# erwincoumans/tiny-differentiable-simulator

Hardware: NVIDIA H100
Metric: env-steps/sec (N parallel sims) (higher is better)
Workload: dtype f32 (ABA, factorisation, PGS) + f64 (kinematics, inertias, CRBA, Jacobians, LCP rhs)

## Files before the change

### tiny-differentiable-simulator_b200/csrc/tds_steps.cu

```cuda
#include <cuda_runtime.h>
#include <stdlib.h>

#include "tds_wcommon.cuh"
#include "tds_team.h"
#include "generated/spec_laikago.h"
#include "generated/spec_ant.h"

namespace tdss {
using namespace tds;
using namespace tdsw;

#ifndef TDS_DENSE_MAX_CAND
#define TDS_DENSE_MAX_CAND 8
#endif
constexpr int TT = TDS_TEAM_T;
constexpr int ST = 32;

template <int V> struct IC { static constexpr int value = V; };
#define CI(...) (IC<(__VA_ARGS__)>::value)
#define CD(...) ([]() { constexpr double cd_v_ = (__VA_ARGS__); return cd_v_; }())
#define CDOT3(ax, ay, az, v)                                                                                            \
  ([&]() {                                                                                                              \
    using T_ = decltype((v).x);                                                                                         \
    constexpr double a_ = (ax), b_ = (ay), c_ = (az);                                                                   \
// ... 171 lines not shown
template <class SP> struct CandTab {
  static constexpr int NC = SP::N_CAND > 0 ? SP::N_CAND : 1;
  int owner[NC], own[NC];
};
template <class SP> constexpr CandTab<SP> make_cand() {
  CandTab<SP> t{};
  for (int g = 0; g < SP::N_CAND; ++g) {
    t.owner[g] = SP::CAND_OWNER[g];
    t.own[g] = (SP::CAND_OWNER[g] == 0 && SP::CAND_LPT[g] < Cls<SP>::n_pts_trunk()) ? 0 : 1;
  }
  return t;
}
template <class SP> __device__ const CandTab<SP>& cand_tab();

template <class SP, typename RA, typename RC, typename RS> struct Lay {
  static constexpr int RAW = sizeof(RA) / 4, RCW = sizeof(RC) / 4, RSW = sizeof(RS) / 4;
  static constexpr int NTD = SP::N_TD, NTRI = NTD * (NTD + 1) / 2, NOD = SP::N_OD_MAX;
  static constexpr int O = 0;
  static constexpr int RB = O + 4 * RCW;
  static constexpr int XWW = ev(12 * RCW + 12 * RAW);
  static constexpr int XW = RB + 10 * RCW;
  static constexpr int TS = XW + (SP::N_XW_TEAM + 1) * XWW;
  static constexpr int TLW = ev(14 * RAW);
  static constexpr int TL = TS + SP::N_TRUNK * 6 * RCW;
  static constexpr int TLR = ev(TL + SP::N_TRUNK * TLW);
  static constexpr int TKS = ev(TLR + trunk_rbi_slot<SP>(SP::N_TRUNK) * 10 * RCW);
  static constexpr int TQD = ev(TKS + 3 * SP::N_TRUNK);
  static constexpr int ACC_IC = ev(27 * RAW);
  static constexpr int ACCW = ev(ACC_IC + 10 * RCW);
  static constexpr int ACC = ev(TQD + NTD);
  static constexpr int PW = ev(NTRI * RSW);
  static constexpr int CONW = ev((3 * (NOD + NTD) + 9) * RSW);
  static constexpr int ACC_SZ = cmax(cmax(TT * cmax(SP::N_ATT, 1) * ACCW, TT * PW), cmax(SP::N_CAND, 1) * CONW);
  static constexpr int LT = ACC + ACC_SZ;
  static constexpr int CON = ACC;
  static constexpr int ZT = ev(LT + NTRI * RSW);
  static constexpr int WO = ev(ZT + NTD * RSW);
  static constexpr int ASTG = ev(WO + TT * NOD * RSW);
  static constexpr int XS = ev(ASTG + SP::N_ACT);
  static constexpr int FLG = ev(XS + (SP::N_CAND > TDS_DENSE_MAX_CAND ? 3 * SP::N_CAND * RSW : 0));
  static constexpr int SHARED = ev(FLG + 2 * TT + 2);
  static constexpr int PRIV = ev(cmax(SP::KMAX - SP::N_TRUNK, 1) * 10 * RCW);
  static constexpr int TOTAL = SHARED + TT * PRIV;
};

template <typename T> TDS_D T* sp(char* base, int lane, int word) {
  return (sizeof(T) == 4) ? ((T*)base) + (size_t)word * ST + lane : ((T*)base) + (size_t)(word >> 1) * ST + lane;
}
template <typename T> TDS_D T negz() { return T(-0.0); }
template <typename T> TDS_D Abi<T> abi_nz() {
  Abi<T> a; const T z = negz<T>();
  a.I = {z, z, z, z, z, z}; a.M = a.I;
// ... 19 lines not shown
  using L = Lay<SP, RA, RC, RS>;
  using C = Cls<SP>;
  static_assert(C::uniform(), "the subtrees of the model are not one structural class (use the table-driven kernel)");
  constexpr bool XOUT = VAR == 0, HOSTIO = VAR == 2;
  constexpr int RAW = L::RAW, RCW = L::RCW;
  constexpr int NT = SP::N_TRUNK, NTD = SP::N_TD, NLOC = SP::N_LOC[0];
  constexpr int NOD = SP::N_OD[0], NODA = cmax(NOD, 1), NTDA = cmax(NTD, 1), NTRI = L::NTRI, NTRIA = cmax(NTRI, 1);
  constexpr int NPO = C::n_pts_own(), NPOA = cmax(NPO, 1), NPTR = C::n_pts_trunk(), NPTRA = cmax(NPTR, 1);
  constexpr int NACCA = cmax(SP::N_ACC, 1), NXLA = cmax(SP::N_XW_LANE, 1), NATT = cmax(SP::N_ATT, 1);
  constexpr bool FLOAT = SP::FLOATING != 0;
  const int lane = tid & 31;
  const int env = tile * 32 + lane;
  const bool live = env < io.n;
  const int e = live ? env : io.n - 1;
  const int ns = io.n_stride;
  const LegTab<SP>& LG = leg_tab<SP>(role);
  char* const priv = smem + (size_t)(L::SHARED + role * L::PRIV) * ST * 4;
  int phase_id = 0;
#define TDSS_PHASE() do { if (io.phase_clk && lane == 0 && tile * 32 < io.n_stride) io.phase_clk[((size_t)tile * TT + role) * 16 + phase_id] = clock64(); ++phase_id; } while (0)
#define TDSS_STAMP(slot) do { if (io.phase_clk && lane == 0 && tile * 32 < io.n_stride) io.phase_clk[((size_t)tile * TT + role) * 16 + (slot)] = clock64(); } while (0)
  TDSS_PHASE();
  auto xw_rc = [&](int slot) { return sp<RC>(smem, lane, L::XW + slot * L::XWW); };
  auto xw_ra = [&](int slot) { return sp<RA>(smem, lane, L::XW + slot * L::XWW + 12 * RCW); };
  auto tl_rbi_slot = [&](int slot) { return sp<RC>(smem, lane, L::TLR + slot * 10 * RCW); };
  auto tl_u = [&](int k) { return sp<RA>(smem, lane, L::TL + k * L::TLW); };
  auto tl_v = [&](int k) { return sp<RA>(smem, lane, L::TL + k * L::TLW + 8 * RAW); };
  auto ts_S = [&](int k) { return sp<RC>(smem, lane, L::TS + k * 6 * RCW); };
  float* const tqd = sp<float>(smem, lane, L::TQD);
  unsigned* const flg = sp<unsigned>(smem, lane, L::FLG);

  float qv[SP::KMAX], qdv[SP::KMAX], tauv[SP::KMAX];
  float bq[7], bqd[6];
  sfor<NT, NLOC>([&](auto Kc) {
    constexpr int k = decltype(Kc)::value;
    if constexpr (!(C::flags(k) & TDS_LF_FIXED)) {
      qv[k] = io.q_in[(size_t)LG.qidx[k - NT] * ns + e];
      qdv[k] = io.qd_in[(size_t)LG.qdidx[k - NT] * ns + e];
      tauv[k] = 0.f;
    }
  });
  if (role == 0) {
    sfor<0, NT>([&](auto Kc) {
      constexpr int k = decltype(Kc)::value;
      if constexpr (!(SP::L_FLAGS[0][k] & TDS_LF_FIXED)) {
        qv[k] = io.q_in[(size_t)CI(SP::L_QIDX[0][k]) * ns + e];
        qdv[k] = io.qd_in[(size_t)CI(SP::L_QDIDX[0][k]) * ns + e];
        tauv[k] = 0.f;
      }
    });
    if constexpr (FLOAT) {
// ... 189 lines not shown
      };
      if constexpr ((fl & TDS_LF_PRISMATIC) != 0) {
        const V3<RC> d = rot_axis();
        pi = axpy(d, qi, pi);
        S.bot = d;
      } else {
        const V3<RC> w = rot_axis();
        if constexpr (jt == TDSJ_REVOLUTE_AXIS) {
          const RC dl = sqrt_t(dot(axv, axv));
          RC s = snv[k] / dl;
          const RC c = csv[k];
          Ri = mul(Ri, quat_to_matrix<RC>(axv.x * s, axv.y * s, axv.z * s, c));
        } else {
          const RC s = snv[k], c = csv[k];
          const V3<RC> cx = col_x(Ri), cy = col_y(Ri), cz = col_z(Ri);
          if constexpr (jt == TDSJ_REVOLUTE_X) set_cols(Ri, cx, axpy(cz, s, cy * c), axpy(cy, -s, cz * c));
          else if constexpr (jt == TDSJ_REVOLUTE_Y) set_cols(Ri, axpy(cz, -s, cx * c), cy, axpy(cx, s, cz * c));
          else set_cols(Ri, axpy(cy, s, cx * c), axpy(cx, -s, cy * c), cz);
        }
        S.top = w;
        S.bot = cross(pi, w);
      }
    }
    if constexpr (TR) st6<RC>(ts_S(k), ST, S); else Sreg[k] = S;
    {
      constexpr bool massless = TR ? (SP::L_RBIC[0][k][0] == 0.0 && SP::L_RBIC[0][k][4] == 0.0 && SP::L_RBIC[0][k][5] == 0.0 && SP::L_RBIC[0][k][6] == 0.0 &&
                                      SP::L_RBIC[0][k][7] == 0.0 && SP::L_RBIC[0][k][8] == 0.0 && SP::L_RBIC[0][k][9] == 0.0)
                                   : C::massless(k);
      if constexpr (!massless) {
        double b[10];
        if constexpr (TR) {
          b[0] = CD(SP::L_RBIC[0][k][0]); b[1] = CD(SP::L_RBIC[0][k][1]); b[2] = CD(SP::L_RBIC[0][k][2]); b[3] = CD(SP::L_RBIC[0][k][3]); b[4] = CD(SP::L_RBIC[0][k][4]);
          b[5] = CD(SP::L_RBIC[0][k][5]); b[6] = CD(SP::L_RBIC[0][k][6]); b[7] = CD(SP::L_RBIC[0][k][7]); b[8] = CD(SP::L_RBIC[0][k][8]); b[9] = CD(SP::L_RBIC[0][k][9]);
        } else {
#pragma unroll
          for (int j = 0; j < 10; ++j) b[j] = LG.rbic[ko][j];
        }
        Rbi<RC> r;
        r.m = RC(b[0]);
        const V3<RC> c = pi + mul(Ri, v3<RC>(RC(b[1]), RC(b[2]), RC(b[3])));
        r.h = c * r.m;
        S3<RA> Icf;
        Icf.xx = RA(b[4]); Icf.xy = RA(b[5]); Icf.xz = RA(b[6]); Icf.yy = RA(b[7]); Icf.yz = RA(b[8]); Icf.zz = RA(b[9]);
        const S3<RA> Irot = rot_sym(cvt<RA>(Ri), Icf);
        r.I.xx = RC(Irot.xx); r.I.xy = RC(Irot.xy); r.I.xz = RC(Irot.xz); r.I.yy = RC(Irot.yy); r.I.yz = RC(Irot.yz); r.I.zz = RC(Irot.zz);
        const RC cc = dot(c, c);
        r.I.xx += r.m * (cc - c.x * c.x); r.I.yy += r.m * (cc - c.y * c.y); r.I.zz += r.m * (cc - c.z * c.z);
        r.I.xy -= r.m * c.x * c.y; r.I.xz -= r.m * c.x * c.z; r.I.yz -= r.m * c.y * c.z;
        if constexpr (TR) st_rbi<RC>(tl_rbi_slot(trunk_rbi_slot<SP>(k)), ST, r);
        else st_rbi<RC>(sp<RC>(priv, lane, ko * 10 * RCW), ST, r);
      }
    }
    Sv<RA> v = vp;
    if constexpr (!(fl & TDS_LF_FIXED)) {
      const RA qdi = RA(qdv[k]);
      const Sv<RA> Sf = cvt_sv<RA>(S);
      v.top = axpy(Sf.top, qdi, v.top);
      v.bot = axpy(Sf.bot, qdi, v.bot);
    }
    if constexpr (TR) st6<RA>(tl_v(k), ST, v); else vreg[k] = v;
    constexpr int xs = SP::L_XW[0][k];
    if constexpr (xs >= 0) {
      if constexpr (TR) { st9<RC>(xw_rc(xs + 1), ST, Ri); st3<RC>(xw_rc(xs + 1) + 9 * ST, ST, pi); st6<RA>(xw_ra(xs + 1), ST, v); }
      else { xwR[xs] = Ri; xwp[xs] = pi; }
    }
    if (want_contacts) {
      if constexpr (TR) emit_trunk_geoms(IC<SP::L_GB[0][k]>{}, IC<SP::L_GE[0][k]>{}, IC<SP::L_CAND[0][k]>{}, IC<SP::L_LPT[0][k]>{}, Ri, pi);
      else emit_own_geoms(IC<k>{}, Ri, pi);
    }
    if constexpr (XOUT) if (io.link_xf && live) {
      int link;
      if constexpr (TR) link = CI(SP::L_LINK[0][k]); else link = LG.link[ko];
      float* o = io.link_xf + (size_t)link * 12 * ns + e;
      o[0] = (float)Ri.xx; o[(size_t)1 * ns] = (float)Ri.xy; o[(size_t)2 * ns] = (float)Ri.xz;
      o[(size_t)3 * ns] = (float)Ri.yx; o[(size_t)4 * ns] = (float)Ri.yy; o[(size_t)5 * ns] = (float)Ri.yz;
      o[(size_t)6 * ns] = (float)Ri.zx; o[(size_t)7 * ns] = (float)Ri.zy; o[(size_t)8 * ns] = (float)Ri.zz;
      o[(size_t)9 * ns] = (float)(pi.x + O.x); o[(size_t)10 * ns] = (float)(pi.y + O.y); o[(size_t)11 * ns] = (float)(pi.z + O.z);
    }
    R_prev = Ri; p_prev = pi; v_prev = v;
// ... 28 lines not shown
          }
        }
      });
    }
    plane_off = DOT_PN(O) - RC(CD(SP::PLANE_C[0]));
    st3<RC>(sO, ST, O); sO[3 * ST] = plane_off;
    if constexpr (FLOAT) st9<RC>(sRb, ST, Rb0);
    R_prev = Rb0;
    p_prev = FLOAT ? v3<RC>(RC(0), RC(0), RC(0)) : v3<RC>(-O.x, -O.y, -O.z);
    if constexpr (FLOAT) {
      const M3<RA> RbA = cvt<RA>(Rb0);
      v_prev.top = mul(RbA, v3<RA>(RA(bqd[0]), RA(bqd[1]), RA(bqd[2])));
      v_prev.bot = mul(RbA, v3<RA>(RA(bqd[3]), RA(bqd[4]), RA(bqd[5])));
    } else { v_prev.top = v3<RA>(RA(0), RA(0), RA(0)); v_prev.bot = v_prev.top; }
    st9<RC>(xw_rc(0), ST, R_prev); st3<RC>(xw_rc(0) + 9 * ST, ST, p_prev); st6<RA>(xw_ra(0), ST, v_prev);
    if (want_contacts) emit_trunk_geoms(IC<SP::GEOM_BEGIN[0]>{}, IC<SP::GEOM_BEGIN[1]>{}, IC<0>{}, IC<0>{}, R_prev, p_prev);
    sfor<0, NT>(pass1);
    TDSS_STAMP(13);
  }
  __syncthreads();
  O = ld3<RC>(sO, ST); plane_off = sO[3 * ST];
  M3<RC> Rb = m3_identity<RC>();
  if constexpr (FLOAT) Rb = ld9<RC>(sRb, ST);
  sfor<NT, NLOC>(pass1);
  flg[(2 * role) * ST] = (unsigned)my_active;
  flg[(2 * role + 1) * ST] = (unsigned)(my_active >> 32);
  if constexpr (HOSTIO) {
#pragma unroll
    for (int j = 0; j < AREG; ++j) {
      const int idx = tid + 32 * TT * j;
      if (idx < NACT_TILE) astg[idx] = areg[j];
    }
  }
  const bool cta_contact = __syncthreads_or(my_active != 0ull) != 0;
  if constexpr (HOSTIO) {
    pd_torques();
    if constexpr (TRUNK_LOOP && !DIRECT_TRUNK) {
      if (role == 0) {
        sfor<0, NT>([&](auto Kc) {
          constexpr int k = decltype(Kc)::value;
          if constexpr (!(SP::L_FLAGS[0][k] & TDS_LF_FIXED)) tk_tau[k * ST] = tauv[k];
        });
      }
    }
  }
  const bool solve = (mode == MODE_FULL) && cta_contact;
// ... 2 lines not shown
  for (int r = 0; r < TT; ++r) team_active |= ((unsigned long long)flg[(2 * r + 1) * ST] << 32) | flg[(2 * r) * ST];
  TDSS_PHASE();

  constexpr int NMKK = NODA * (NODA + 1) / 2, NCM = NODA * NTDA;
  RS Mkk[NMKK];
#ifdef TDS_STEPS_KERNEL_ONLY
  RS Cm_store[NCM];
  RS* const Cm = Cm_store;
#else
  RS Cm[NCM];
#endif
  RS Bm[NTRIA];
#pragma unroll
  for (int i = 0; i < NMKK; ++i) Mkk[i] = RS(0);
#pragma unroll
  for (int i = 0; i < NCM; ++i) Cm[i] = RS(0);
#pragma unroll
  for (int i = 0; i < NTRIA; ++i) Bm[i] = RS(0);
  Sv<RA> Ureg[SP::KMAX]; RA invDreg[SP::KMAX], ureg[SP::KMAX];
  Abi<RA> cA = abi_nz<RA>(); Sv<RA> cP = sv_nz<RA>(); Rbi<RC> cC = rbi_nz<RC>();
  Abi<RA> accA[NACCA]; Sv<RA> accP[NACCA]; Rbi<RC> accC[NACCA];
#pragma unroll
  for (int s = 0; s < NACCA; ++s) { accA[s] = abi_nz<RA>(); accP[s] = sv_nz<RA>(); accC[s] = rbi_nz<RC>(); }
  auto S_of = [&](auto Jc) -> Sv<RC> {
    constexpr int j = decltype(Jc)::value;
    if constexpr (j < NT) return ld6<RC>(ts_S(j), ST); else return Sreg[j];
  };
  auto acc_ptr_ra = [&](int r, int s) { return sp<RA>(smem, lane, L::ACC + (r * NATT + s) * L::ACCW); };
  auto acc_ptr_rc = [&](int r, int s) { return sp<RC>(smem, lane, L::ACC + (r * NATT + s) * L::ACCW + L::ACC_IC); };
  auto pass2 = [&](auto Kc) {
    constexpr int k = decltype(Kc)::value;
    constexpr bool TR = k < NT;
    constexpr int ko = TR ? 0 : k - NT;
    constexpr int fl = TR ? SP::L_FLAGS[0][k] : C::flags(k);
    constexpr bool massless = TR ? (SP::L_RBIC[0][k][0] == 0.0 && SP::L_RBIC[0][k][4] == 0.0 && SP::L_RBIC[0][k][5] == 0.0 && SP::L_RBIC[0][k][6] == 0.0 &&
                                    SP::L_RBIC[0][k][7] == 0.0 && SP::L_RBIC[0][k][8] == 0.0 && SP::L_RBIC[0][k][9] == 0.0)
                                 : C::massless(k);
    Sv<RA> v;
    if constexpr (TR) v = ld6<RA>(tl_v(k), ST); else v = vreg[k];
    Rbi<RC> Ic = rbi_nz<RC>();
    Abi<RA> Ia = abi_nz<RA>();
    Sv<RA> pA = sv_nz<RA>();
    if constexpr (!massless) {
      if constexpr (TR) Ic = ld_rbi<RC>(tl_rbi_slot(trunk_rbi_slot<SP>(k)), ST); else Ic = ld_rbi<RC>(sp<RC>(priv, lane, ko * 10 * RCW), ST);
      const Rbi<RA> rb = cvt_rbi<RA>(Ic);
      Ia = abi_from_rbi(rb);
      pA = cross_mf(v, rbi_mul(rb, v));
    }
    if constexpr ((fl & TDS_TF_CHILD_ADJ) != 0) { abi_add(Ia, cA); pA = pA + cP; rbi_add(Ic, cC); }
    constexpr int as = SP::L_ACC[0][k];
    if constexpr (as >= 0) {
      abi_add(Ia, accA[as]); pA = pA + accP[as]; rbi_add(Ic, accC[as]);
      if constexpr (as < SP::N_ATT) {
        static_assert(TR || k < 0, "attachment accumulators are consumed by trunk links");
        sfor<1, TT>([&](auto Rc_) {
          constexpr int r = decltype(Rc_)::value;
          Abi<RA> sa; Sv<RA> sv_;
          acc_ld27<RA>(acc_ptr_ra(r, as), ST, sa, sv_);
          abi_add(Ia, sa); pA = pA + sv_;
          rbi_add(Ic, ld_rbi<RC>(acc_ptr_rc(r, as), ST));
        });
      }
    }
    Sv<RA> pa = pA;
    if constexpr (!(fl & TDS_LF_FIXED)) {
      const Sv<RC> Sd = S_of(IC<k>{});
      const Sv<RA> S = cvt_sv<RA>(Sd);
      const RA qdj = RA(qdv[k]);
      Sv<RA> vJ; vJ.top = S.top * qdj; vJ.bot = S.bot * qdj;
      const Sv<RA> c = cross_mm(v, vJ);
      const Sv<RA> U = abi_mul(Ia, S);
      const RA D = dot(S, U);
      const RA invD = inv_t(D);
      RA tau = RA(tauv[k]);
      if constexpr (TR) {
        if constexpr (SP::L_SD[0][k][0] != 0.0) tau -= RA(CD(SP::L_SD[0][k][0])) * RA(qv[k]);
        if constexpr (SP::L_SD[0][k][1] != 0.0) tau -= RA(CD(SP::L_SD[0][k][1])) * qdj;
      } else {
        if constexpr (C::has_sd(k, 0)) tau -= RA(LG.sd[ko][0]) * RA(qv[k]);
        if constexpr (C::has_sd(k, 1)) tau -= RA(LG.sd[ko][1]) * qdj;
      }
      const RA u = tau - dot(S, pA);
      if constexpr (TR) { st6<RA>(tl_v(k), ST, c); st6<RA>(tl_u(k), ST, U); tl_u(k)[6 * ST] = invD; tl_u(k)[7 * ST] = u; }
      else { vreg[k] = c; Ureg[k] = U; invDreg[k] = invD; ureg[k] = u; }
      const V3<RA> ut = U.top * invD, ub = U.bot * invD;
      Ia.I.xx -= U.top.x * ut.x; Ia.I.xy -= U.top.x * ut.y; Ia.I.xz -= U.top.x * ut.z;
      Ia.I.yy -= U.top.y * ut.y; Ia.I.yz -= U.top.y * ut.z; Ia.I.zz -= U.top.z * ut.z;
      Ia.H.xx -= U.top.x * ub.x; Ia.H.xy -= U.top.x * ub.y; Ia.H.xz -= U.top.x * ub.z;
      Ia.H.yx -= U.top.y * ub.x; Ia.H.yy -= U.top.y * ub.y; Ia.H.yz -= U.top.y * ub.z;
      Ia.H.zx -= U.top.z * ub.x; Ia.H.zy -= U.top.z * ub.y; Ia.H.zz -= U.top.z * ub.z;
      Ia.M.xx -= U.bot.x * ub.x; Ia.M.xy -= U.bot.x * ub.y; Ia.M.xz -= U.bot.x * ub.z;
      Ia.M.yy -= U.bot.y * ub.y; Ia.M.yz -= U.bot.y * ub.z; Ia.M.zz -= U.bot.z * ub.z;
      const Sv<RA> Iac = abi_mul(Ia, c);
      const RA uD = u * invD;
      pa.top = pA.top + Iac.top + U.top * uD;
      pa.bot = pA.bot + Iac.bot + U.bot * uD;
      if (solve) {
        const Sv<RC> F = rbi_mul(Ic, Sd);
        const RS mii = RS(dot(Sd, F));
        constexpr int ld = SP::L_LDOF[0][k];
        if constexpr (TR) Bm[tri(ld, ld)] = mii; else Mkk[tri(ld - NTD, ld - NTD)] = mii;
        sfor<0, k>([&](auto Jc) {
          constexpr int j = decltype(Jc)::value;
          constexpr int lj = SP::L_LDOF[0][j];
          if constexpr (lj >= 0 && is_anc<SP, 0>(j, k)) {
            const RS val = RS(dot(S_of(IC<j>{}), F));
            if constexpr (TR) Bm[tri(ld, lj)] = val;
            else if constexpr (lj >= NTD) Mkk[tri(ld - NTD, lj - NTD)] = val;
            else Cm[(ld - NTD) * NTDA + lj] = val;
          }
        });
        if constexpr (FLOAT) {
          const V3<RC> ft = mulT(Rb, F.top), fb = mulT(Rb, F.bot);
          if constexpr (TR) {
            Bm[tri(ld, 0)] = RS(ft.x); Bm[tri(ld, 1)] = RS(ft.y); Bm[tri(ld, 2)] = RS(ft.z);
            Bm[tri(ld, 3)] = RS(fb.x); Bm[tri(ld, 4)] = RS(fb.y); Bm[tri(ld, 5)] = RS(fb.z);
          } else {
            RS* row = Cm + (ld - NTD) * NTDA;
            row[0] = RS(ft.x); row[1] = RS(ft.y); row[2] = RS(ft.z); row[3] = RS(fb.x); row[4] = RS(fb.y); row[5] = RS(fb.z);
          }
        }
      }
    }
    if constexpr ((fl & TDS_TF_PARENT_ADJ) != 0) { cA = Ia; cP = pa; cC = Ic; }
    else {
      constexpr int slot = SP::L_PAR[0][k];
      if constexpr (slot >= 0) { abi_add(accA[slot], Ia); accP[slot] = accP[slot] + pa; rbi_add(accC[slot], Ic); }
    }
  };
  sfor_rev<NT, NLOC>(pass2);
  if (TRUNK_LOOP || role != 0) {
    sfor<0, SP::N_ATT>([&](auto Sc) {
      constexpr int s = decltype(Sc)::value;
      RA* pa_ = acc_ptr_ra(role, s);
      const Abi<RA>& a = accA[s]; const Sv<RA>& f = accP[s];
      pa_[0] = a.I.xx; pa_[ST] = a.I.xy; pa_[2 * ST] = a.I.xz; pa_[3 * ST] = a.I.yy; pa_[4 * ST] = a.I.yz; pa_[5 * ST] = a.I.zz;
      pa_[6 * ST] = a.H.xx; pa_[7 * ST] = a.H.xy; pa_[8 * ST] = a.H.xz; pa_[9 * ST] = a.H.yx; pa_[10 * ST] = a.H.yy; pa_[11 * ST] = a.H.yz;
      pa_[12 * ST] = a.H.zx; pa_[13 * ST] = a.H.zy; pa_[14 * ST] = a.H.zz;
      pa_[15 * ST] = a.M.xx; pa_[16 * ST] = a.M.xy; pa_[17 * ST] = a.M.xz; pa_[18 * ST] = a.M.yy; pa_[19 * ST] = a.M.yz; pa_[20 * ST] = a.M.zz;
      pa_[21 * ST] = f.top.x; pa_[22 * ST] = f.top.y; pa_[23 * ST] = f.top.z; pa_[24 * ST] = f.bot.x; pa_[25 * ST] = f.bot.y; pa_[26 * ST] = f.bot.z;
      st_rbi<RC>(acc_ptr_rc(role, s), ST, accC[s]);
    });
  }
  __syncthreads();
  TDSS_STAMP(10);

  const RA dtA = RA(P.dt);
  Sv<RA> a_prev;
  auto pass3 = [&](auto Kc) {
    constexpr int k = decltype(Kc)::value;
    constexpr bool TR = k < NT;
    constexpr int ko = TR ? 0 : k - NT;
    constexpr int fl = TR ? SP::L_FLAGS[0][k] : C::flags(k), lpar = SP::L_LPAR[0][k];
    Sv<RA> a;
    if constexpr ((fl & TDS_TF_PARENT_ADJ) != 0) a = a_prev;
    else if constexpr (lpar < NT) {
      constexpr int slot = lpar < 0 ? 0 : SP::L_XW[0][lpar < 0 ? 0 : lpar] + 1;
      a = ld6<RA>(xw_ra(slot) + 6 * ST, ST);
    } else a = xwa[CI(SP::L_XW[0][lpar < NT ? NT : lpar])];
    if constexpr (!(fl & TDS_LF_FIXED)) {
      Sv<RA> c, U; RA invD, u;
      if constexpr (TR) { c = ld6<RA>(tl_v(k), ST); U = ld6<RA>(tl_u(k), ST); invD = tl_u(k)[6 * ST]; u = tl_u(k)[7 * ST]; }
      else { c = vreg[k]; U = Ureg[k]; invD = invDreg[k]; u = ureg[k]; }
      a = a + c;
      const RA qdd = invD * (u - dot(U, a));
      const Sv<RA> S = cvt_sv<RA>(S_of(IC<k>{}));
      a.top = axpy(S.top, qdd, a.top);
      a.bot = axpy(S.bot, qdd, a.bot);
      if (XOUT && mode == MODE_FD) {
        if (live && io.qdd_out) {
          int qdi;
          if constexpr (TR) qdi = CI(SP::L_QDIDX[0][k]); else qdi = LG.qdidx[ko];
          io.qdd_out[(size_t)qdi * ns + e] = (float)qdd;
        }
      } else qdv[k] = (float)(RA(qdv[k]) + qdd * dtA);
    }
    constexpr int xs = SP::L_XW[0][k];
    if constexpr (xs >= 0) {
      if constexpr (TR) st6<RA>(xw_ra(xs + 1) + 6 * ST, ST, a); else xwa[xs] = a;
    }
    a_prev = a;
  };
  if constexpr (CRBA_HELPERS) {
    if (role != 0 && solve) {
      const TrunkTab<SP>& TK = trunk_tab<SP>();
      RS* const Bs = sp<RS>(smem, lane, L::LT);
      Rbi<RC> Ic = rbi_nz<RC>();
#pragma unroll 1
      for (int k = NT - 1; k >= 0; --k) {
        if (!TK.massless[k]) rbi_add(Ic, ld_rbi<RC>(tl_rbi_slot(TK.rbi_slot[k]), ST));
        const int as = TK.acc[k];
        if (as >= 0) {
#pragma unroll
          for (int r = 0; r < TT; ++r) rbi_add(Ic, ld_rbi<RC>(acc_ptr_rc(r, as), ST));
        }
        if (!TK.fixed[k] && (k % (TT - 1)) == role - 1) {
          const Sv<RC> Sd = ld6<RC>(ts_S(k), ST);
          const Sv<RC> F = rbi_mul(Ic, Sd);
          const int ld = TK.ldof[k];
          RS* const brow = Bs + (size_t)(ld * (ld + 1) / 2) * ST;
          brow[ld * ST] = RS(dot(Sd, F));
#pragma unroll
          for (int j = 0; j < NT - 1; ++j) {
            const int lj = TK.ldof[j];
            if (j < k && lj >= 0) brow[lj * ST] = RS(dot(ld6<RC>(ts_S(j), ST), F));
          }
          if constexpr (FLOAT) {
            const V3<RC> ft = mulT(Rb, F.top), fb = mulT(Rb, F.bot);
            brow[0] = RS(ft.x); brow[ST] = RS(ft.y); brow[2 * ST] = RS(ft.z);
            brow[3 * ST] = RS(fb.x); brow[4 * ST] = RS(fb.y); brow[5 * ST] = RS(fb.z);
          }
        }
      }
    }
  }
  if (role == 0) {
    if constexpr (DIRECT_TRUNK) {
    } else if constexpr (TRUNK_LOOP) {
      const TrunkTab<SP>& TK = trunk_tab<SP>();
      RS* const Bs = sp<RS>(smem, lane, L::LT);
      cA = abi_nz<RA>(); cP = sv_nz<RA>(); cC = rbi_nz<RC>();
#pragma unroll 1
      for (int k = NT - 1; k >= 0; --k) {
        const Sv<RA> v = ld6<RA>(tl_v(k), ST);
        Rbi<RC> Ic = cC; Abi<RA> Ia = cA; Sv<RA> pA = cP;
        if (!TK.massless[k]) {
          const Rbi<RC> own = ld_rbi<RC>(tl_rbi_slot(TK.rbi_slot[k]), ST);
          const Rbi<RA> rb = cvt_rbi<RA>(own);
          abi_add(Ia, abi_from_rbi(rb));
          pA = pA + cross_mf(v, rbi_mul(rb, v));
          rbi_add(Ic, own);
        }
        const int as = TK.acc[k];
        if (as >= 0) {
#pragma unroll
          for (int r = 0; r < TT; ++r) {
            Abi<RA> sa; Sv<RA> sv_;
            acc_ld27<RA>(acc_ptr_ra(r, as), ST, sa, sv_);
            abi_add(Ia, sa); pA = pA + sv_;
            rbi_add(Ic, ld_rbi<RC>(acc_ptr_rc(r, as), ST));
          }
        }
        Sv<RA> pa = pA;
        if (!TK.fixed[k]) {
          const Sv<RC> Sd = ld6<RC>(ts_S(k), ST);
          const Sv<RA> S = cvt_sv<RA>(Sd);
          const RA qdj = RA(tk_qd[k * ST]);
          Sv<RA> vJ; vJ.top = S.top * qdj; vJ.bot = S.bot * qdj;
          const Sv<RA> c = cross_mm(v, vJ);
          const Sv<RA> U = abi_mul(Ia, S);
          const RA D = dot(S, U);
          const RA invD = inv_t(D);
          RA tau = RA(tk_tau[k * ST]);
          tau -= RA(TK.sd[k][0]) * RA(tk_q[k * ST]);
          tau -= RA(TK.sd[k][1]) * qdj;
          const RA u = tau - dot(S, pA);
          st6<RA>(tl_v(k), ST, c); st6<RA>(tl_u(k), ST, U); tl_u(k)[6 * ST] = invD; tl_u(k)[7 * ST] = u;
          const V3<RA> ut = U.top * invD, ub = U.bot * invD;
          Ia.I.xx -= U.top.x * ut.x; Ia.I.xy -= U.top.x * ut.y; Ia.I.xz -= U.top.x * ut.z;
          Ia.I.yy -= U.top.y * ut.y; Ia.I.yz -= U.top.y * ut.z; Ia.I.zz -= U.top.z * ut.z;
          Ia.H.xx -= U.top.x * ub.x; Ia.H.xy -= U.top.x * ub.y; Ia.H.xz -= U.top.x * ub.z;
          Ia.H.yx -= U.top.y * ub.x; Ia.H.yy -= U.top.y * ub.y; Ia.H.yz -= U.top.y * ub.z;
          Ia.H.zx -= U.top.z * ub.x; Ia.H.zy -= U.top.z * ub.y; Ia.H.zz -= U.top.z * ub.z;
          Ia.M.xx -= U.bot.x * ub.x; Ia.M.xy -= U.bot.x * ub.y; Ia.M.xz -= U.bot.x * ub.z;
          Ia.M.yy -= U.bot.y * ub.y; Ia.M.yz -= U.bot.y * ub.z; Ia.M.zz -= U.bot.z * ub.z;
          const Sv<RA> Iac = abi_mul(Ia, c);
          const RA uD = u * invD;
          pa.top = pA.top + Iac.top + U.top * uD;
          pa.bot = pA.bot + Iac.bot + U.bot * uD;
          if (solve && !CRBA_HELPERS) {
            const Sv<RC> F = rbi_mul(Ic, Sd);
            const int ld = TK.ldof[k];
            RS* const brow = Bs + (size_t)(ld * (ld + 1) / 2) * ST;
            brow[ld * ST] = RS(dot(Sd, F));
#pragma unroll
            for (int j = 0; j < NT - 1; ++j) {
              const int lj = TK.ldof[j];
              if (j < k && lj >= 0) brow[lj * ST] = RS(dot(ld6<RC>(ts_S(j), ST), F));
            }
            if constexpr (FLOAT) {
              const V3<RC> ft = mulT(Rb, F.top), fb = mulT(Rb, F.bot);
              brow[0] = RS(ft.x); brow[ST] = RS(ft.y); brow[2 * ST] = RS(ft.z);
              brow[3 * ST] = RS(fb.x); brow[4 * ST] = RS(fb.y); brow[5 * ST] = RS(fb.z);
            }
          }
        }
        cA = Ia; cP = pa; cC = Ic;
      }
    } else sfor_rev<0, NT>(pass2);
    TDSS_STAMP(11);
    Sv<RC> base_acc_b; base_acc_b.top = v3<RC>(RC(0), RC(0), RC(0)); base_acc_b.bot = base_acc_b.top;
    if constexpr (FLOAT) {
      Abi<RA> Ach = abi_nz<RA>(); Sv<RA> pch = sv_nz<RA>(); Rbi<RC> Icch = rbi_nz<RC>();
      if constexpr (NT > 0) {
        if constexpr (SP::L_LPAR[0][0] < 0 && (SP::L_FLAGS[0][0] & TDS_TF_PARENT_ADJ) != 0) { abi_add(Ach, cA); pch = pch + cP; rbi_add(Icch, cC); }
      }
      if constexpr (SP::BASE_SLOT >= 0) {
        constexpr int as = SP::BASE_SLOT;
        abi_add(Ach, accA[as]); pch = pch + accP[as]; rbi_add(Icch, accC[as]);
        if constexpr (as < SP::N_ATT) {
          sfor<1, TT>([&](auto Rc_) {
            constexpr int r = decltype(Rc_)::value;
            Abi<RA> sa; Sv<RA> sv_;
            acc_ld27<RA>(acc_ptr_ra(r, as), ST, sa, sv_);
            abi_add(Ach, sa); pch = pch + sv_;
            rbi_add(Icch, ld_rbi<RC>(acc_ptr_rc(r, as), ST));
          });
        }
      }
      const M3<RA> Rt = cvt<RA>(transpose(Rb));
      Abi<RA> Ab;
      {
        Rbi<RA> rbb; rbb.m = RA(CD(SP::BASE_RBI[0])); rbb.h = v3<RA>(RA(CD(SP::BASE_RBI[1])), RA(CD(SP::BASE_RBI[2])), RA(CD(SP::BASE_RBI[3])));
        rbb.I = {RA(CD(SP::BASE_RBI[4])), RA(CD(SP::BASE_RBI[5])), RA(CD(SP::BASE_RBI[6])), RA(CD(SP::BASE_RBI[7])), RA(CD(SP::BASE_RBI[8])), RA(CD(SP::BASE_RBI[9]))};
        Ab = abi_from_rbi(rbb);
        Abi<RA> Arot;
        Arot.I = rot_sym(Rt, Ach.I); Arot.M = rot_sym(Rt, Ach.M); Arot.H = rot_gen(Rt, Ach.H);
        abi_add(Ab, Arot);
      }
      Sv<RA> pb;
      {
        const M3<RA> RbA = cvt<RA>(Rb);
        M3<RA> Ic0;
        Ic0.xx = RA((float)CD(SP::BASE_INERTIA_COM[0])); Ic0.xy = RA((float)CD(SP::BASE_INERTIA_COM[1])); Ic0.xz = RA((float)CD(SP::BASE_INERTIA_COM[2]));
        Ic0.yx = RA((float)CD(SP::BASE_INERTIA_COM[3])); Ic0.yy = RA((float)CD(SP::BASE_INERTIA_COM[4])); Ic0.yz = RA((float)CD(SP::BASE_INERTIA_COM[5]));
        Ic0.zx = RA((float)CD(SP::BASE_INERTIA_COM[6])); Ic0.zy = RA((float)CD(SP::BASE_INERTIA_COM[7])); Ic0.zz = RA((float)CD(SP::BASE_INERTIA_COM[8]));
        const M3<RA> Iw = rot_gen(RbA, Ic0);
        const V3<RA> wb = v3<RA>(RA(bqd[0]), RA(bqd[1]), RA(bqd[2]));
        pb.top = cross(wb, mul(Iw, wb)) + mul(Rt, pch.top);
// ... 34 lines not shown
        M3<RC> Cn = neg(H3);
        M3<RC> Dm = inv3(sub(M3m, mul(mul(Cn, Ainv), H3)));
        M3<RC> AinvBD = mul(mul(Ainv, H3), Dm);
        M3<RC> Ii = add(Ainv, mul(mul(AinvBD, Cn), Ainv));
        M3<RC> Hi = neg(AinvBD);
        V3<RC> ft = cvt<RC>(pb.top), fb = cvt<RC>(pb.bot);
        V3<RC> at = mul(Ii, ft) + mul(Hi, fb);
        V3<RC> ab = mul(Dm, fb) + mulT(Hi, ft);
        base_acc_b.top = v3<RC>(-at.x, -at.y, -at.z);
        base_acc_b.bot = v3<RC>(-ab.x, -ab.y, -ab.z);
      }
      a_prev.top = cvt<RA>(mul(Rb, base_acc_b.top));
      a_prev.bot = cvt<RA>(mul(Rb, base_acc_b.bot));
    } else {
      a_prev.top = v3<RA>(RA(0), RA(0), RA(0));
      a_prev.bot = v3<RA>(RA(-P.gravity[0]), RA(-P.gravity[1]), RA(-P.gravity[2]));
    }
    st6<RA>(xw_ra(0) + 6 * ST, ST, a_prev);
    if constexpr (DIRECT_TRUNK) {
      constexpr int kb = NT - 1;
      const Sv<RA> v_b = ld6<RA>(tl_v(kb), ST);
      Abi<RA> Ia = abi_nz<RA>(); Sv<RA> pA = sv_nz<RA>();
      if constexpr (!trunk_massless<SP>(kb)) {
        const Rbi<RA> rb = cvt_rbi<RA>(ld_rbi<RC>(tl_rbi_slot(trunk_rbi_slot<SP>(kb)), ST));
        Ia = abi_from_rbi(rb);
        pA = cross_mf(v_b, rbi_mul(rb, v_b));
      }
      constexpr int as = SP::L_ACC[0][kb];
      if constexpr (as >= 0) {
        sfor<0, TT>([&](auto Rc_) {
          constexpr int r = decltype(Rc_)::value;
          Abi<RA> sa; Sv<RA> sv_;
          acc_ld27<RA>(acc_ptr_ra(r, as), ST, sa, sv_);
          abi_add(Ia, sa); pA = pA + sv_;
        });
      }
      Sv<RA> Sk[NT], Uk[NT];
      Sv<RA> acc = a_prev;
      sfor<0, NT>([&](auto Kc) {
        constexpr int k = decltype(Kc)::value;
        Sk[k] = cvt_sv<RA>(ld6<RC>(ts_S(k), ST));
        const RA qdk = RA(qdv[k]);
        Sv<RA> vJ; vJ.top = Sk[k].top * qdk; vJ.bot = Sk[k].bot * qdk;
        acc = acc + cross_mm(ld6<RA>(tl_v(k), ST), vJ);
        Uk[k] = abi_mul(Ia, Sk[k]);
      });
      const Sv<RA> w = abi_mul(Ia, acc) + pA;
      RA Dm[NT * (NT + 1) / 2], x[NT];
      sfor<0, NT>([&](auto Ic_) {
        constexpr int i = decltype(Ic_)::value;
        x[i] = RA(tauv[i]) - dot(Sk[i], w);
        sfor<0, i + 1>([&](auto Jc) { constexpr int j = decltype(Jc)::value; Dm[tri(i, j)] = dot(Sk[i], Uk[j]); });
      });
      sfor<0, NT>([&](auto Ic_) {
        constexpr int i = decltype(Ic_)::value;
        sfor<0, i + 1>([&](auto Jc) {
          constexpr int j = decltype(Jc)::value;
          RA sacc = Dm[tri(i, j)];
          sfor<0, j>([&](auto Kc) { constexpr int k = decltype(Kc)::value; sacc -= Dm[tri(i, k)] * Dm[tri(j, k)]; });
          if constexpr (j < i) Dm[tri(i, j)] = sacc * Dm[tri(j, j)];
          else Dm[tri(i, i)] = rsqrt_t(sacc);
        });
        RA sy = x[i];
        sfor<0, i>([&](auto Kc) { constexpr int k = decltype(Kc)::value; sy -= Dm[tri(i, k)] * x[k]; });
// ... 7 lines not shown
      });
      Sv<RA> a = acc;
      sfor<0, NT>([&](auto Kc) {
        constexpr int k = decltype(Kc)::value;
        const RA qdd = x[k];
        a.top = axpy(Sk[k].top, qdd, a.top);
        a.bot = axpy(Sk[k].bot, qdd, a.bot);
        if (XOUT && mode == MODE_FD) { if (live && io.qdd_out) io.qdd_out[(size_t)CI(SP::L_QDIDX[0][k]) * ns + e] = (float)qdd; }
        else qdv[k] = (float)(RA(qdv[k]) + qdd * dtA);
      });
      constexpr int xsb = SP::L_XW[0][kb];
      if constexpr (xsb >= 0) st6<RA>(xw_ra(xsb + 1) + 6 * ST, ST, a);
      a_prev = a;
    } else if constexpr (TRUNK_LOOP) {
      const TrunkTab<SP>& TK = trunk_tab<SP>();
      Sv<RA> a = a_prev;
#pragma unroll 1
      for (int k = 0; k < NT; ++k) {
        if (!TK.fixed[k]) {
          const Sv<RA> c = ld6<RA>(tl_v(k), ST), U = ld6<RA>(tl_u(k), ST);
          const RA invD = tl_u(k)[6 * ST], u = tl_u(k)[7 * ST];
          a = a + c;
          const RA qdd = invD * (u - dot(U, a));
          const Sv<RA> S = cvt_sv<RA>(ld6<RC>(ts_S(k), ST));
          a.top = axpy(S.top, qdd, a.top);
          a.bot = axpy(S.bot, qdd, a.bot);
          if (XOUT && mode == MODE_FD) { if (live && io.qdd_out) io.qdd_out[(size_t)TK.qdidx[k] * ns + e] = (float)qdd; }
          else tk_qd[k * ST] = (float)(RA(tk_qd[k * ST]) + qdd * dtA);
        }
        const int xs = TK.xw[k];
        if (xs >= 0) st6<RA>(xw_ra(xs + 1) + 6 * ST, ST, a);
      }
      a_prev = a;
      sfor<0, NT>([&](auto Kc) {
        constexpr int k = decltype(Kc)::value;
        if constexpr (!(SP::L_FLAGS[0][k] & TDS_LF_FIXED)) qdv[k] = tk_qd[k * ST];
      });
    } else sfor<0, NT>(pass3);
    if constexpr (FLOAT) {
      const RC qb[6] = {base_acc_b.top.x, base_acc_b.top.y, base_acc_b.top.z, base_acc_b.bot.x + RC(P.gravity[0]),
                        base_acc_b.bot.y + RC(P.gravity[1]), base_acc_b.bot.z + RC(P.gravity[2])};
#pragma unroll
      for (int k = 0; k < 6; ++k) {
        if (XOUT && mode == MODE_FD) { if (live && io.qdd_out) io.qdd_out[(size_t)k * ns + e] = (float)qb[k]; }
        else bqd[k] = (float)(RC(bqd[k]) + qb[k] * RC(P.dt));
      }
#pragma unroll
// ... 75 lines not shown
#pragma unroll
      for (int i = 0; i < BB + 9; ++i) row[i * ST] = RS(0);
    };
    auto point_rows = [&](auto Kl, const int cand, const V3<RC>& xc, const RC dist) {
      constexpr int kl = decltype(Kl)::value;
      RS ro[3][NODA], rt[3][NTDA];
#pragma unroll
      for (int d = 0; d < 3; ++d) {
#pragma unroll
        for (int i = 0; i < NODA; ++i) ro[d][i] = RS(0);
#pragma unroll
        for (int i = 0; i < NTDA; ++i) rt[d][i] = RS(0);
      }
      V3<RC> vel = v3<RC>(RC(0), RC(0), RC(0));
      if constexpr (FLOAT) {
        const V3<RC> cols[6] = {v3<RC>(RC(0), -xc.z, xc.y), v3<RC>(xc.z, RC(0), -xc.x), v3<RC>(-xc.y, xc.x, RC(0)),
                                v3<RC>(RC(1), RC(0), RC(0)), v3<RC>(RC(0), RC(1), RC(0)), v3<RC>(RC(0), RC(0), RC(1))};
#pragma unroll
        for (int k = 0; k < 6; ++k) {
          rt[0][k] = RS(DOT_NB(cols[k])); rt[1][k] = RS(DOT_F1(cols[k])); rt[2][k] = RS(DOT_F2(cols[k]));
          vel = vel + cols[k] * RC(tqd[k * ST]);
        }
      }
      sfor<0, (kl < 0 ? 0 : kl + 1)>([&](auto Jc) {
        constexpr int j = decltype(Jc)::value;
        constexpr int lj = SP::L_LDOF[0][j];
        if constexpr (lj >= 0 && (j == kl || is_anc<SP, 0>(j, kl))) {
          const Sv<RC> S = S_of(IC<j>{});
          const V3<RC> col = S.bot + cross(S.top, xc);
          const RS c0 = RS(DOT_NB(col)), c1 = RS(DOT_F1(col)), c2 = RS(DOT_F2(col));
          if constexpr (lj >= NTD) { ro[0][lj - NTD] = c0; ro[1][lj - NTD] = c1; ro[2][lj - NTD] = c2; vel = vel + col * RC(qdv[j]); }
          else { rt[0][lj] = c0; rt[1][lj] = c1; rt[2][lj] = c2; vel = vel + col * RC(tqd[lj * ST]); }
        }
      });
      RS* const row = sp<RS>(smem, lane, L::CON) + (size_t)cand * (L::CONW / L::RSW) * ST;
      row[(BB + 0) * ST] = RS((RC(1) + RC(P.restitution)) * DOT_NB(vel) - RC(P.erp) * dist * RC(P.inv_dt));
      row[(BB + 1) * ST] = RS(DOT_F1(vel));
      row[(BB + 2) * ST] = RS(DOT_F2(vel));
#pragma unroll
      for (int d = 0; d < 3; ++d) {
        RS yy = RS(0);
        if constexpr (kl >= NT) {
          sfor<0, NOD>([&](auto Ic_) {
            constexpr int i = decltype(Ic_)::value;
            RS s = ro[d][i];
            sfor<0, i>([&](auto Kc) { constexpr int k = decltype(Kc)::value; s -= Mkk[tri(i, k)] * ro[d][k]; });
            ro[d][i] = s * Mkk[tri(i, i)];
// ... 484 lines not shown
```

Measured before the change: 370.5 million.

## Store trunk motion subspaces and composite inertias in f32 shared memory

Trunk joint motion subspaces, trunk rigid-body inertias and the accumulated composite inertias passed between team roles are now kept in shared memory in the ABA float type instead of double. The trunk CRBA loops, Jacobian rows and contact velocity contributions are computed in float. This shrinks the shared-memory layout and removes double arithmetic and double-width loads on the hot trunk paths. The cost is lower precision in the mass matrix and the contact Jacobian entries, which the workload description lists as f64 parts.

```diff
diff --git a/tiny-differentiable-simulator_b200/csrc/tds_steps.cu b/tiny-differentiable-simulator_b200/csrc/tds_steps.cu
--- a/tiny-differentiable-simulator_b200/csrc/tds_steps.cu
+++ b/tiny-differentiable-simulator_b200/csrc/tds_steps.cu
@@ -1,5 +1,7 @@
 #include <cuda_runtime.h>
 #include <stdlib.h>
+
+#include <type_traits>
 
 #include "tds_wcommon.cuh"
 #include "tds_team.h"
@@ -217,12 +219,12 @@
   static constexpr int XW = RB + 10 * RCW;
   static constexpr int TS = XW + (SP::N_XW_TEAM + 1) * XWW;
   static constexpr int TLW = ev(14 * RAW);
-  static constexpr int TL = TS + SP::N_TRUNK * 6 * RCW;
+  static constexpr int TL = TS + SP::N_TRUNK * 6 * RAW;
   static constexpr int TLR = ev(TL + SP::N_TRUNK * TLW);
-  static constexpr int TKS = ev(TLR + trunk_rbi_slot<SP>(SP::N_TRUNK) * 10 * RCW);
+  static constexpr int TKS = ev(TLR + trunk_rbi_slot<SP>(SP::N_TRUNK) * 10 * RAW);
   static constexpr int TQD = ev(TKS + 3 * SP::N_TRUNK);
   static constexpr int ACC_IC = ev(27 * RAW);
-  static constexpr int ACCW = ev(ACC_IC + 10 * RCW);
+  static constexpr int ACCW = ev(ACC_IC + 10 * RAW);
   static constexpr int ACC = ev(TQD + NTD);
   static constexpr int PW = ev(NTRI * RSW);
   static constexpr int CONW = ev((3 * (NOD + NTD) + 9) * RSW);
@@ -288,10 +290,10 @@
   TDSS_PHASE();
   auto xw_rc = [&](int slot) { return sp<RC>(smem, lane, L::XW + slot * L::XWW); };
   auto xw_ra = [&](int slot) { return sp<RA>(smem, lane, L::XW + slot * L::XWW + 12 * RCW); };
-  auto tl_rbi_slot = [&](int slot) { return sp<RC>(smem, lane, L::TLR + slot * 10 * RCW); };
+  auto tl_rbi_slot = [&](int slot) { return sp<RA>(smem, lane, L::TLR + slot * 10 * RAW); };
   auto tl_u = [&](int k) { return sp<RA>(smem, lane, L::TL + k * L::TLW); };
   auto tl_v = [&](int k) { return sp<RA>(smem, lane, L::TL + k * L::TLW + 8 * RAW); };
-  auto ts_S = [&](int k) { return sp<RC>(smem, lane, L::TS + k * 6 * RCW); };
+  auto ts_S = [&](int k) { return sp<RA>(smem, lane, L::TS + k * 6 * RAW); };
   float* const tqd = sp<float>(smem, lane, L::TQD);
   unsigned* const flg = sp<unsigned>(smem, lane, L::FLG);
 
@@ -527,7 +529,8 @@
         S.bot = cross(pi, w);
       }
     }
-    if constexpr (TR) st6<RC>(ts_S(k), ST, S); else Sreg[k] = S;
+    const Sv<RA> Sf = cvt_sv<RA>(S);
+    if constexpr (TR) st6<RA>(ts_S(k), ST, Sf); else Sreg[k] = S;
     {
       constexpr bool massless = TR ? (SP::L_RBIC[0][k][0] == 0.0 && SP::L_RBIC[0][k][4] == 0.0 && SP::L_RBIC[0][k][5] == 0.0 && SP::L_RBIC[0][k][6] == 0.0 &&
                                       SP::L_RBIC[0][k][7] == 0.0 && SP::L_RBIC[0][k][8] == 0.0 && SP::L_RBIC[0][k][9] == 0.0)
@@ -541,25 +544,25 @@
 #pragma unroll
           for (int j = 0; j < 10; ++j) b[j] = LG.rbic[ko][j];
         }
-        Rbi<RC> r;
-        r.m = RC(b[0]);
-        const V3<RC> c = pi + mul(Ri, v3<RC>(RC(b[1]), RC(b[2]), RC(b[3])));
+        using T = typename std::conditional<TR, RA, RC>::type;
+        Rbi<T> r;
+        r.m = T(b[0]);
+        const V3<T> c = cvt<T>(pi) + mul(cvt<T>(Ri), v3<T>(T(b[1]), T(b[2]), T(b[3])));
         r.h = c * r.m;
         S3<RA> Icf;
         Icf.xx = RA(b[4]); Icf.xy = RA(b[5]); Icf.xz = RA(b[6]); Icf.yy = RA(b[7]); Icf.yz = RA(b[8]); Icf.zz = RA(b[9]);
         const S3<RA> Irot = rot_sym(cvt<RA>(Ri), Icf);
-        r.I.xx = RC(Irot.xx); r.I.xy = RC(Irot.xy); r.I.xz = RC(Irot.xz); r.I.yy = RC(Irot.yy); r.I.yz = RC(Irot.yz); r.I.zz = RC(Irot.zz);
-        const RC cc = dot(c, c);
+        r.I.xx = T(Irot.xx); r.I.xy = T(Irot.xy); r.I.xz = T(Irot.xz); r.I.yy = T(Irot.yy); r.I.yz = T(Irot.yz); r.I.zz = T(Irot.zz);
+        const T cc = dot(c, c);
         r.I.xx += r.m * (cc - c.x * c.x); r.I.yy += r.m * (cc - c.y * c.y); r.I.zz += r.m * (cc - c.z * c.z);
         r.I.xy -= r.m * c.x * c.y; r.I.xz -= r.m * c.x * c.z; r.I.yz -= r.m * c.y * c.z;
-        if constexpr (TR) st_rbi<RC>(tl_rbi_slot(trunk_rbi_slot<SP>(k)), ST, r);
+        if constexpr (TR) st_rbi<RA>(tl_rbi_slot(trunk_rbi_slot<SP>(k)), ST, r);
         else st_rbi<RC>(sp<RC>(priv, lane, ko * 10 * RCW), ST, r);
       }
     }
     Sv<RA> v = vp;
     if constexpr (!(fl & TDS_LF_FIXED)) {
       const RA qdi = RA(qdv[k]);
-      const Sv<RA> Sf = cvt_sv<RA>(S);
       v.top = axpy(Sf.top, qdi, v.top);
       v.bot = axpy(Sf.bot, qdi, v.bot);
     }
@@ -634,6 +637,7 @@
   O = ld3<RC>(sO, ST); plane_off = sO[3 * ST];
   M3<RC> Rb = m3_identity<RC>();
   if constexpr (FLOAT) Rb = ld9<RC>(sRb, ST);
+  const M3<RA> RbA = cvt<RA>(Rb);
   sfor<NT, NLOC>(pass1);
   flg[(2 * role) * ST] = (unsigned)my_active;
   flg[(2 * role + 1) * ST] = (unsigned)(my_active >> 32);
@@ -682,12 +686,12 @@
   Abi<RA> accA[NACCA]; Sv<RA> accP[NACCA]; Rbi<RC> accC[NACCA];
 #pragma unroll
   for (int s = 0; s < NACCA; ++s) { accA[s] = abi_nz<RA>(); accP[s] = sv_nz<RA>(); accC[s] = rbi_nz<RC>(); }
-  auto S_of = [&](auto Jc) -> Sv<RC> {
+  auto S_of = [&](auto Jc) {
     constexpr int j = decltype(Jc)::value;
-    if constexpr (j < NT) return ld6<RC>(ts_S(j), ST); else return Sreg[j];
+    if constexpr (j < NT) return ld6<RA>(ts_S(j), ST); else return Sreg[j];
   };
   auto acc_ptr_ra = [&](int r, int s) { return sp<RA>(smem, lane, L::ACC + (r * NATT + s) * L::ACCW); };
-  auto acc_ptr_rc = [&](int r, int s) { return sp<RC>(smem, lane, L::ACC + (r * NATT + s) * L::ACCW + L::ACC_IC); };
+  auto acc_ptr_ic = [&](int r, int s) { return sp<RA>(smem, lane, L::ACC + (r * NATT + s) * L::ACCW + L::ACC_IC); };
   auto pass2 = [&](auto Kc) {
     constexpr int k = decltype(Kc)::value;
     constexpr bool TR = k < NT;
@@ -702,7 +706,7 @@
     Abi<RA> Ia = abi_nz<RA>();
     Sv<RA> pA = sv_nz<RA>();
     if constexpr (!massless) {
-      if constexpr (TR) Ic = ld_rbi<RC>(tl_rbi_slot(trunk_rbi_slot<SP>(k)), ST); else Ic = ld_rbi<RC>(sp<RC>(priv, lane, ko * 10 * RCW), ST);
+      if constexpr (TR) Ic = cvt_rbi<RC>(ld_rbi<RA>(tl_rbi_slot(trunk_rbi_slot<SP>(k)), ST)); else Ic = ld_rbi<RC>(sp<RC>(priv, lane, ko * 10 * RCW), ST);
       const Rbi<RA> rb = cvt_rbi<RA>(Ic);
       Ia = abi_from_rbi(rb);
       pA = cross_mf(v, rbi_mul(rb, v));
@@ -718,14 +722,15 @@
           Abi<RA> sa; Sv<RA> sv_;
           acc_ld27<RA>(acc_ptr_ra(r, as), ST, sa, sv_);
           abi_add(Ia, sa); pA = pA + sv_;
-          rbi_add(Ic, ld_rbi<RC>(acc_ptr_rc(r, as), ST));
+          rbi_add(Ic, cvt_rbi<RC>(ld_rbi<RA>(acc_ptr_ic(r, as), ST)));
         });
       }
     }
     Sv<RA> pa = pA;
     if constexpr (!(fl & TDS_LF_FIXED)) {
-      const Sv<RC> Sd = S_of(IC<k>{});
-      const Sv<RA> S = cvt_sv<RA>(Sd);
+      const auto Sk_ = S_of(IC<k>{});
+      const Sv<RC> Sd = cvt_sv<RC>(Sk_);
+      const Sv<RA> S = cvt_sv<RA>(Sk_);
       const RA qdj = RA(qdv[k]);
       Sv<RA> vJ; vJ.top = S.top * qdj; vJ.bot = S.bot * qdj;
       const Sv<RA> c = cross_mm(v, vJ);
@@ -757,6 +762,7 @@
       pa.bot = pA.bot + Iac.bot + U.bot * uD;
       if (solve) {
         const Sv<RC> F = rbi_mul(Ic, Sd);
+        const Sv<RA> FA = cvt_sv<RA>(F);
         const RS mii = RS(dot(Sd, F));
         constexpr int ld = SP::L_LDOF[0][k];
         if constexpr (TR) Bm[tri(ld, ld)] = mii; else Mkk[tri(ld - NTD, ld - NTD)] = mii;
@@ -764,7 +770,8 @@
           constexpr int j = decltype(Jc)::value;
           constexpr int lj = SP::L_LDOF[0][j];
           if constexpr (lj >= 0 && is_anc<SP, 0>(j, k)) {
-            const RS val = RS(dot(S_of(IC<j>{}), F));
+            RS val;
+            if constexpr (j < NT) val = RS(dot(S_of(IC<j>{}), FA)); else val = RS(dot(S_of(IC<j>{}), F));
             if constexpr (TR) Bm[tri(ld, lj)] = val;
             else if constexpr (lj >= NTD) Mkk[tri(ld - NTD, lj - NTD)] = val;
             else Cm[(ld - NTD) * NTDA + lj] = val;
@@ -799,7 +806,7 @@
       pa_[12 * ST] = a.H.zx; pa_[13 * ST] = a.H.zy; pa_[14 * ST] = a.H.zz;
       pa_[15 * ST] = a.M.xx; pa_[16 * ST] = a.M.xy; pa_[17 * ST] = a.M.xz; pa_[18 * ST] = a.M.yy; pa_[19 * ST] = a.M.yz; pa_[20 * ST] = a.M.zz;
       pa_[21 * ST] = f.top.x; pa_[22 * ST] = f.top.y; pa_[23 * ST] = f.top.z; pa_[24 * ST] = f.bot.x; pa_[25 * ST] = f.bot.y; pa_[26 * ST] = f.bot.z;
-      st_rbi<RC>(acc_ptr_rc(role, s), ST, accC[s]);
+      st_rbi<RA>(acc_ptr_ic(role, s), ST, cvt_rbi<RA>(accC[s]));
     });
   }
   __syncthreads();
@@ -845,28 +852,28 @@
     if (role != 0 && solve) {
       const TrunkTab<SP>& TK = trunk_tab<SP>();
       RS* const Bs = sp<RS>(smem, lane, L::LT);
-      Rbi<RC> Ic = rbi_nz<RC>();
+      Rbi<RA> Ic = rbi_nz<RA>();
 #pragma unroll 1
       for (int k = NT - 1; k >= 0; --k) {
-        if (!TK.massless[k]) rbi_add(Ic, ld_rbi<RC>(tl_rbi_slot(TK.rbi_slot[k]), ST));
+        if (!TK.massless[k]) rbi_add(Ic, ld_rbi<RA>(tl_rbi_slot(TK.rbi_slot[k]), ST));
         const int as = TK.acc[k];
         if (as >= 0) {
 #pragma unroll
-          for (int r = 0; r < TT; ++r) rbi_add(Ic, ld_rbi<RC>(acc_ptr_rc(r, as), ST));
+          for (int r = 0; r < TT; ++r) rbi_add(Ic, ld_rbi<RA>(acc_ptr_ic(r, as), ST));
         }
         if (!TK.fixed[k] && (k % (TT - 1)) == role - 1) {
-          const Sv<RC> Sd = ld6<RC>(ts_S(k), ST);
-          const Sv<RC> F = rbi_mul(Ic, Sd);
+          const Sv<RA> S = ld6<RA>(ts_S(k), ST);
+          const Sv<RA> F = rbi_mul(Ic, S);
           const int ld = TK.ldof[k];
           RS* const brow = Bs + (size_t)(ld * (ld + 1) / 2) * ST;
-          brow[ld * ST] = RS(dot(Sd, F));
+          brow[ld * ST] = RS(dot(S, F));
 #pragma unroll
           for (int j = 0; j < NT - 1; ++j) {
             const int lj = TK.ldof[j];
-            if (j < k && lj >= 0) brow[lj * ST] = RS(dot(ld6<RC>(ts_S(j), ST), F));
+            if (j < k && lj >= 0) brow[lj * ST] = RS(dot(ld6<RA>(ts_S(j), ST), F));
           }
           if constexpr (FLOAT) {
-            const V3<RC> ft = mulT(Rb, F.top), fb = mulT(Rb, F.bot);
+            const V3<RA> ft = mulT(RbA, F.top), fb = mulT(RbA, F.bot);
             brow[0] = RS(ft.x); brow[ST] = RS(ft.y); brow[2 * ST] = RS(ft.z);
             brow[3 * ST] = RS(fb.x); brow[4 * ST] = RS(fb.y); brow[5 * ST] = RS(fb.z);
           }
@@ -879,16 +886,16 @@
     } else if constexpr (TRUNK_LOOP) {
       const TrunkTab<SP>& TK = trunk_tab<SP>();
       RS* const Bs = sp<RS>(smem, lane, L::LT);
-      cA = abi_nz<RA>(); cP = sv_nz<RA>(); cC = rbi_nz<RC>();
+      cA = abi_nz<RA>(); cP = sv_nz<RA>();
+      Rbi<RA> cCa = rbi_nz<RA>();
 #pragma unroll 1
       for (int k = NT - 1; k >= 0; --k) {
         const Sv<RA> v = ld6<RA>(tl_v(k), ST);
-        Rbi<RC> Ic = cC; Abi<RA> Ia = cA; Sv<RA> pA = cP;
+        Rbi<RA> Ic = cCa; Abi<RA> Ia = cA; Sv<RA> pA = cP;
         if (!TK.massless[k]) {
-          const Rbi<RC> own = ld_rbi<RC>(tl_rbi_slot(TK.rbi_slot[k]), ST);
-          const Rbi<RA> rb = cvt_rbi<RA>(own);
-          abi_add(Ia, abi_from_rbi(rb));
-          pA = pA + cross_mf(v, rbi_mul(rb, v));
+          const Rbi<RA> own = ld_rbi<RA>(tl_rbi_slot(TK.rbi_slot[k]), ST);
+          abi_add(Ia, abi_from_rbi(own));
+          pA = pA + cross_mf(v, rbi_mul(own, v));
           rbi_add(Ic, own);
         }
         const int as = TK.acc[k];
@@ -898,13 +905,12 @@
             Abi<RA> sa; Sv<RA> sv_;
             acc_ld27<RA>(acc_ptr_ra(r, as), ST, sa, sv_);
             abi_add(Ia, sa); pA = pA + sv_;
-            rbi_add(Ic, ld_rbi<RC>(acc_ptr_rc(r, as), ST));
+            rbi_add(Ic, ld_rbi<RA>(acc_ptr_ic(r, as), ST));
           }
         }
         Sv<RA> pa = pA;
         if (!TK.fixed[k]) {
-          const Sv<RC> Sd = ld6<RC>(ts_S(k), ST);
-          const Sv<RA> S = cvt_sv<RA>(Sd);
+          const Sv<RA> S = ld6<RA>(ts_S(k), ST);
           const RA qdj = RA(tk_qd[k * ST]);
           Sv<RA> vJ; vJ.top = S.top * qdj; vJ.bot = S.bot * qdj;
           const Sv<RA> c = cross_mm(v, vJ);
@@ -929,24 +935,25 @@
           pa.top = pA.top + Iac.top + U.top * uD;
           pa.bot = pA.bot + Iac.bot + U.bot * uD;
           if (solve && !CRBA_HELPERS) {
-            const Sv<RC> F = rbi_mul(Ic, Sd);
+            const Sv<RA> F = rbi_mul(Ic, S);
             const int ld = TK.ldof[k];
             RS* const brow = Bs + (size_t)(ld * (ld + 1) / 2) * ST;
-            brow[ld * ST] = RS(dot(Sd, F));
+            brow[ld * ST] = RS(dot(S, F));
 #pragma unroll
             for (int j = 0; j < NT - 1; ++j) {
               const int lj = TK.ldof[j];
-              if (j < k && lj >= 0) brow[lj * ST] = RS(dot(ld6<RC>(ts_S(j), ST), F));
+              if (j < k && lj >= 0) brow[lj * ST] = RS(dot(ld6<RA>(ts_S(j), ST), F));
             }
             if constexpr (FLOAT) {
-              const V3<RC> ft = mulT(Rb, F.top), fb = mulT(Rb, F.bot);
+              const V3<RA> ft = mulT(RbA, F.top), fb = mulT(RbA, F.bot);
               brow[0] = RS(ft.x); brow[ST] = RS(ft.y); brow[2 * ST] = RS(ft.z);
               brow[3 * ST] = RS(fb.x); brow[4 * ST] = RS(fb.y); brow[5 * ST] = RS(fb.z);
             }
           }
         }
-        cA = Ia; cP = pa; cC = Ic;
-      }
+        cA = Ia; cP = pa; cCa = Ic;
+      }
+      if constexpr (FLOAT) cC = cvt_rbi<RC>(cCa);
     } else sfor_rev<0, NT>(pass2);
     TDSS_STAMP(11);
     Sv<RC> base_acc_b; base_acc_b.top = v3<RC>(RC(0), RC(0), RC(0)); base_acc_b.bot = base_acc_b.top;
@@ -964,7 +971,7 @@
             Abi<RA> sa; Sv<RA> sv_;
             acc_ld27<RA>(acc_ptr_ra(r, as), ST, sa, sv_);
             abi_add(Ach, sa); pch = pch + sv_;
-            rbi_add(Icch, ld_rbi<RC>(acc_ptr_rc(r, as), ST));
+            rbi_add(Icch, cvt_rbi<RC>(ld_rbi<RA>(acc_ptr_ic(r, as), ST)));
           });
         }
       }
@@ -1045,7 +1052,7 @@
       const Sv<RA> v_b = ld6<RA>(tl_v(kb), ST);
       Abi<RA> Ia = abi_nz<RA>(); Sv<RA> pA = sv_nz<RA>();
       if constexpr (!trunk_massless<SP>(kb)) {
-        const Rbi<RA> rb = cvt_rbi<RA>(ld_rbi<RC>(tl_rbi_slot(trunk_rbi_slot<SP>(kb)), ST));
+        const Rbi<RA> rb = ld_rbi<RA>(tl_rbi_slot(trunk_rbi_slot<SP>(kb)), ST);
         Ia = abi_from_rbi(rb);
         pA = cross_mf(v_b, rbi_mul(rb, v_b));
       }
@@ -1062,7 +1069,7 @@
       Sv<RA> acc = a_prev;
       sfor<0, NT>([&](auto Kc) {
         constexpr int k = decltype(Kc)::value;
-        Sk[k] = cvt_sv<RA>(ld6<RC>(ts_S(k), ST));
+        Sk[k] = ld6<RA>(ts_S(k), ST);
         const RA qdk = RA(qdv[k]);
         Sv<RA> vJ; vJ.top = Sk[k].top * qdk; vJ.bot = Sk[k].bot * qdk;
         acc = acc + cross_mm(ld6<RA>(tl_v(k), ST), vJ);
@@ -1116,7 +1123,7 @@
           const RA invD = tl_u(k)[6 * ST], u = tl_u(k)[7 * ST];
           a = a + c;
           const RA qdd = invD * (u - dot(U, a));
-          const Sv<RA> S = cvt_sv<RA>(ld6<RC>(ts_S(k), ST));
+          const Sv<RA> S = ld6<RA>(ts_S(k), ST);
           a.top = axpy(S.top, qdd, a.top);
           a.bot = axpy(S.bot, qdd, a.bot);
           if (XOUT && mode == MODE_FD) { if (live && io.qdd_out) io.qdd_out[(size_t)TK.qdidx[k] * ns + e] = (float)qdd; }
@@ -1238,7 +1245,21 @@
           vel = vel + cols[k] * RC(tqd[k * ST]);
         }
       }
-      sfor<0, (kl < 0 ? 0 : kl + 1)>([&](auto Jc) {
+      constexpr int KE = kl < 0 ? 0 : kl + 1;
+      const V3<RA> xcA = cvt<RA>(xc);
+      V3<RA> velA = cvt<RA>(vel);
+      sfor<0, (KE < NT ? KE : NT)>([&](auto Jc) {
+        constexpr int j = decltype(Jc)::value;
+        constexpr int lj = SP::L_LDOF[0][j];
+        if constexpr (lj >= 0 && (j == kl || is_anc<SP, 0>(j, kl))) {
+          const Sv<RA> S = S_of(IC<j>{});
+          const V3<RA> col = S.bot + cross(S.top, xcA);
+          rt[0][lj] = RS(DOT_NB(col)); rt[1][lj] = RS(DOT_F1(col)); rt[2][lj] = RS(DOT_F2(col));
+          velA = velA + col * RA(tqd[lj * ST]);
+        }
+      });
+      vel = cvt<RC>(velA);
+      sfor<NT, (KE > NT ? KE : NT)>([&](auto Jc) {
         constexpr int j = decltype(Jc)::value;
         constexpr int lj = SP::L_LDOF[0][j];
         if constexpr (lj >= 0 && (j == kl || is_anc<SP, 0>(j, kl))) {
```

Result: slower. 356.2 million, median of 6 (-3.8%).
